# PM25/Information-Retrieval-with-Contrastive-Learning

Hardware: AMD Instinct MI355X
Metric: query-doc pairs/sec (train) + queries/sec @ top-k over N docs, 1/2/4/8 GPU (higher is better)
Workload: dtype bf16

## Files before the change

### information-retrieval-with-contrastive-learning_amd/csrc/gemm.hip

```cpp
#include "gemm_epi.h"
#include "gemm_pp.h"

#include <algorithm>
#include <atomic>
#include <type_traits>

#ifndef IRC_GEMM_GROUP_M
#define IRC_GEMM_GROUP_M 0
#endif

namespace irc {
namespace gemm {

enum Layout { ROW = 0, COL = 1 };

constexpr int BM = 128, BN = 128, NT = 256;

template <typename T>
struct TT;
template <>
struct TT<unsigned short> {
  static constexpr int BK = 32;
  static constexpr int VEC = 8;
  static constexpr int PITCH = BK * 2 + 16;
// ... 1090 lines not shown
        if (EPI == EPI_BIAS_GELU_SAVE) {
          TO* pre = const_cast<TO*>(R) + (int64_t)row * g.ldr + col;
          if constexpr (sizeof(TO) == 2)
            *reinterpret_cast<unsigned short*>(pre) = f32_to_bf16(v);
          else
            *reinterpret_cast<float*>(pre) = v;
          v = gelu_fast(v);
        }
        if (EPI == EPI_BIAS_RESID || EPI == EPI_RESID || EPI == EPI_DGELU) {
          float r;
          if constexpr (sizeof(TO) == 2)
            r = bf16_to_f32(reinterpret_cast<const unsigned short*>(R)[(int64_t)row * g.ldr + col]);
          else
            r = reinterpret_cast<const float*>(R)[(int64_t)row * g.ldr + col];
          v = EPI == EPI_DGELU ? v * gelu_grad_fast(r) : v + r;
        }
        TO* dst = C + (int64_t)row * g.ldc + col;
        if constexpr (sizeof(TO) == 2) {
          *reinterpret_cast<unsigned short*>(dst) = f32_to_bf16(v);
        } else {
          if (g.accumulate)
            *reinterpret_cast<float*>(dst) += v;
          else
            *reinterpret_cast<float*>(dst) = v;
        }
      }
    }
  }
}

typedef __bf16 bf16x2_v __attribute__((ext_vector_type(2)));
struct QaArgs {
  const unsigned short* x;
  const unsigned short* w;
  const float* bias;
  const int64_t* mask;
  unsigned short* ctx;
  int M, K, H;
  int64_t ldx, ldc;
  float scale;
  int L;
  int group_m;
  int big_dma;
  int l2_touch;
};

template <int SL>
__global__ __launch_bounds__(big::NT, 1) void qkv_attn_kernel(QaArgs g) {
  constexpr bool PACK = SL == 0;
  constexpr int WNB = 3, BM = big::BM, BN = 128 * WNB, TP = BN + 8;
  constexpr int SLX = PACK ? 128 : SL;
  constexpr int SH = SLX == 64 ? 6 : 7;
  constexpr int NJM = SLX / 32;
  __shared__ __attribute__((aligned(1024))) char lds[2 * (BM + BN) * big::ROW_BYTES];
  static_assert(128 * TP * 2 + 8 * SLX * 4 <= 2 * (BM + BN) * big::ROW_BYTES,
                "staged half and mask biases fit the LDS");
  const int nseq = g.M / g.L;
  const int spt = PACK ? BM / g.L : BM / SLX;
  const int ls = PACK || g.L == SL ? 0 : g.L;
  const int tiles_m = (nseq + spt - 1) / spt;
  const int tiles_n = 3 * g.H / BN;
  const int ntiles = tiles_m * tiles_n;
  int bid = blockIdx.x;
  {
    const int q = ntiles / 8, r = ntiles % 8, x = bid % 8;
    bid = (x < r ? x * (q + 1) : r * (q + 1) + (x - r) * q) + bid / 8;
  }
  int tm, tn;
  grouped_tile(bid, tiles_m, tiles_n, g.group_m, tm, tn);
  const int m0 = PACK ? tm * spt * g.L : tm * BM, n0 = tn * BN;
  const int lane = threadIdx.x & 63;
  const int wave = __builtin_amdgcn_readfirstlane(threadIdx.x >> 6);
  const int wm = wave >> 2, wn = wave & 3;
  f32x4 acc4[8][2 * WNB];
#pragma unroll
  for (int i = 0; i < 8; ++i)
#pragma unroll
    for (int j = 0; j < 2 * WNB; ++j) acc4[i][j] = (f32x4)0.0f;
  big::mainloop_mf16<WNB>(g.x, g.ldx, g.w, g.K, m0, n0, g.M, 3 * g.H, g.K, lds, wave, lane, acc4,
                          g.big_dma != 0,
                          big::touch_lines(g.l2_touch, tiles_m, tiles_n, tm, tn, BM, BN), ls, SH);

  unsigned short* T = reinterpret_cast<unsigned short*>(lds);
  float* mbw = reinterpret_cast<float*>(lds + 128 * TP * 2) + SL * wave;
  uint32_t pk[8][2 * WNB][2];
#pragma unroll
  for (int j = 0; j < 2 * WNB; ++j) {
    const int col = n0 + wn * 32 * WNB + 16 * j + (lane & 15);
    const float bvj = g.bias[col];
#pragma unroll
    for (int i = 0; i < 8; ++i)
#pragma unroll
      for (int e2 = 0; e2 < 2; ++e2) {
        f32x2_t v;
#pragma unroll
        for (int u = 0; u < 2; ++u) v[u] = acc4[i][j][2 * e2 + u] * 1.0f + bvj;
        uint32_t w = __builtin_bit_cast(uint32_t, __builtin_convertvector(v, bf16x2_v));
        asm volatile("" : "+v"(w));
        pk[i][j][e2] = w;
      }
  }
  const int h = lane >> 5, r32 = lane & 31;
  const int nj = (g.L + 31) / 32;
  if constexpr (PACK) {
    constexpr int TQ = 264;
    static_assert(BM * TQ * 2 + 8 * 128 * 4 <= 2 * (BM + BN) * big::ROW_BYTES,
                  "staged head and mask biases fit the LDS");
    unsigned short* Tq = reinterpret_cast<unsigned short*>(lds);
    float* mb = reinterpret_cast<float*>(lds + BM * TQ * 2) + 128 * wave;
    const int odd = lane & 1;
    const uint32_t psel = odd ? 0x03020706u : 0x05040100u;
    const int nsq = min(spt, nseq - tm * spt);
    const int nit = nsq * nj;
#pragma unroll
    for (int hd = 0; hd < 2; ++hd) {
#pragma unroll
      for (int j = 0; j < 2 * WNB; ++j) {
        const int b = wn * 32 * WNB + 16 * j;
        if (((b >> 6) & 1) != hd) continue;
        const int tc = 64 * (b >> 7) + (b & 63) + (lane & 14);
#pragma unroll
        for (int i = 0; i < 8; ++i)
#pragma unroll
          for (int e2 = 0; e2 < 2; ++e2) {
            const uint32_t w = pk[i][j][e2];
            const uint32_t x = (uint32_t)__builtin_amdgcn_mov_dpp((int)w, 0xB1, 0xF, 0xF, false);
            const uint32_t v = __builtin_amdgcn_perm(x, w, psel);
            const int rl = 128 * wm + 16 * i + 4 * (lane >> 4) + 2 * e2 + odd;
            *reinterpret_cast<uint32_t*>(&Tq[rl * TQ + tc]) = v;
          }
      }
      __syncthreads();
      for (int it = wave; it < nit; it += 8) {
        const int s = it / nj, ib = it - s * nj;
        const int t0 = s * g.L;
        const int r0 = (tm * spt + s) * g.L;
#pragma unroll
        for (int j = lane; j < 128; j += 64)
          mb[j] = j >= g.L ? -3e30f
                           : ((g.mask == nullptr || g.mask[r0 + j] != 0) ? 0.f : -1e30f);
        const int nkb = visible_key_blocks(g.mask ? g.mask + r0 : nullptr, g.L, nj, lane);
        __builtin_amdgcn_wave_barrier();
        asm volatile("s_waitcnt lgkmcnt(0)" ::: "memory");
        const unsigned short* Q = Tq;
        const unsigned short* Kp = Tq + 64;
        const unsigned short* V = Tq + 128;
        unsigned short* out = g.ctx + (int64_t)r0 * g.ldc + (2 * tn + hd) * 64;
        bf16x8 qf[4];
        const int qr = min(t0 + 32 * ib + r32, BM - 1);
#pragma unroll
        for (int kk = 0; kk < 4; ++kk)
          qf[kk] = *reinterpret_cast<const bf16x8*>(Q + qr * TQ + 16 * kk + 8 * h);
        f32x16 sc[NJM];
#pragma unroll
        for (int jb = 0; jb < NJM; ++jb) {
          sc[jb] = (f32x16)0.f;
          if (jb < nkb) {
            const int kr = min(t0 + 32 * jb + r32, BM - 1);
#pragma unroll
            for (int kk = 0; kk < 4; ++kk) {
              const bf16x8 kf = *reinterpret_cast<const bf16x8*>(Kp + kr * TQ + 16 * kk + 8 * h);
              sc[jb] = __builtin_amdgcn_mfma_f32_32x32x16_bf16(kf, qf[kk], sc[jb], 0, 0, 0);
            }
          }
        }
        float mx = -INFINITY;
#pragma unroll
        for (int jb = 0; jb < NJM; ++jb) {
          if (jb >= nkb) break;
#pragma unroll
          for (int q = 0; q < 4; ++q) {
            const f32x4 bias = *reinterpret_cast<const f32x4*>(&mb[32 * jb + 8 * q + 4 * h]);
#pragma unroll
            for (int r = 0; r < 4; ++r) {
              const float v = sc[jb][4 * q + r] * g.scale + bias[r];
              sc[jb][4 * q + r] = v;
              mx = fmaxf(mx, v);
            }
          }
        }
        mx = fmaxf(mx, __shfl_xor(mx, 32, 64));
        float sum = 0.f;
#pragma unroll
        for (int jb = 0; jb < NJM; ++jb) {
          if (jb >= nkb) break;
#pragma unroll
          for (int e = 0; e < 16; ++e) {
            const float p = __expf(sc[jb][e] - mx);
            sc[jb][e] = p;
            sum += p;
          }
        }
        sum += __shfl_xor(sum, 32, 64);
        const float inv = 1.f / sum;
        f32x16 o[2] = {(f32x16)0.f, (f32x16)0.f};
#pragma unroll
        for (int jb = 0; jb < NJM; ++jb) {
          if (jb >= nkb) break;
#pragma unroll
          for (int k2 = 0; k2 < 2; ++k2) {
            bf16x8 pa;
#pragma unroll
            for (int t = 0; t < 8; ++t) pa[t] = (__bf16)(sc[jb][8 * k2 + t] * inv);
            const int j0 = 32 * jb + 16 * k2 + 4 * h;
            const int i16 = lane & 15;
            const int vr = t0 + j0 + (i16 >> 2);
#pragma unroll
            for (int db = 0; db < 2; ++db) {
              const int vc = 32 * db + 16 * ((lane >> 4) & 1) + 4 * (i16 & 3);
              const v4s lo = ds_tr16(reinterpret_cast<const char*>(V + min(vr, BM - 1) * TQ + vc));
              const v4s hi =
                  ds_tr16(reinterpret_cast<const char*>(V + min(vr + 8, BM - 1) * TQ + vc));
              const v4s both[2] = {lo, hi};
              o[db] = __builtin_amdgcn_mfma_f32_32x32x16_bf16(pa, __builtin_bit_cast(bf16x8, both),
                                                              o[db], 0, 0, 0);
            }
          }
        }
#pragma unroll
        for (int db = 0; db < 2; ++db)
#pragma unroll
          for (int e = 0; e < 16; ++e) {
            const int i = 32 * ib + (e & 3) + 8 * (e >> 2) + 4 * h;
            if (i < g.L) out[(int64_t)i * g.ldc + 32 * db + r32] = f32_to_bf16(o[db][e]);
          }
      }
      if (hd == 0) __syncthreads();
    }
    return;
  }
#pragma unroll
  for (int hf = 0; hf < 2; ++hf) {
    if (wm == hf) {
      const int odd = lane & 1;
      const uint32_t psel = odd ? 0x03020706u : 0x05040100u;
#pragma unroll
      for (int i = 0; i < 8; ++i)
#pragma unroll
        for (int j = 0; j < 2 * WNB; ++j)
#pragma unroll
          for (int e2 = 0; e2 < 2; ++e2) {
            const uint32_t w = pk[i][j][e2];
            const uint32_t x = (uint32_t)__builtin_amdgcn_mov_dpp((int)w, 0xB1, 0xF, 0xF, false);
            const uint32_t v = __builtin_amdgcn_perm(x, w, psel);
            const int rl = 16 * i + 4 * (lane >> 4) + 2 * e2 + odd;
            *reinterpret_cast<uint32_t*>(&T[rl * TP + wn * 32 * WNB + 16 * j + (lane & 14)]) = v;
          }
    }
    __syncthreads();
    const int sl = SL == 64 ? wn >> 1 : 0, hh = SL == 64 ? wn & 1 : wave & 1;
    const int ib = SL == 64 ? wm : wave >> 1;
    const int seq = spt * tm + (SL == 64 ? 2 * hf + sl : hf);
    const int r0 = seq * g.L;
    if (seq < nseq && ib < nj) {
#pragma unroll
      for (int j = lane; j < SL; j += 64)
        mbw[j] = j >= g.L ? -3e30f
                          : ((g.mask == nullptr || g.mask[r0 + j] != 0) ? 0.f : -1e30f);
      const int nkb = visible_key_blocks(g.mask ? g.mask + r0 : nullptr, g.L, nj, lane);
      __builtin_amdgcn_wave_barrier();
      asm volatile("s_waitcnt lgkmcnt(0)" ::: "memory");
      const unsigned short* Ts = T + 64 * sl * TP;
      const unsigned short* Q = Ts + hh * 64;
      const unsigned short* Kp = Ts + 128 + hh * 64;
      const unsigned short* V = Ts + 256 + hh * 64;
      unsigned short* out = g.ctx + (int64_t)r0 * g.ldc + (2 * tn + hh) * 64;
      {
        bf16x8 qf[4];
#pragma unroll
        for (int kk = 0; kk < 4; ++kk)
          qf[kk] = *reinterpret_cast<const bf16x8*>(Q + (32 * ib + r32) * TP + 16 * kk + 8 * h);
        f32x16 sc[NJM];
#pragma unroll
        for (int jb = 0; jb < NJM; ++jb) {
          sc[jb] = (f32x16)0.f;
          if (jb < nkb) {
#pragma unroll
            for (int kk = 0; kk < 4; ++kk) {
              const bf16x8 kf =
                  *reinterpret_cast<const bf16x8*>(Kp + (32 * jb + r32) * TP + 16 * kk + 8 * h);
              sc[jb] = __builtin_amdgcn_mfma_f32_32x32x16_bf16(kf, qf[kk], sc[jb], 0, 0, 0);
            }
          }
        }
        float mx = -INFINITY;
#pragma unroll
        for (int jb = 0; jb < NJM; ++jb) {
          if (jb >= nkb) break;
#pragma unroll
          for (int q = 0; q < 4; ++q) {
            const f32x4 bias = *reinterpret_cast<const f32x4*>(&mbw[32 * jb + 8 * q + 4 * h]);
#pragma unroll
            for (int r = 0; r < 4; ++r) {
              const float v = sc[jb][4 * q + r] * g.scale + bias[r];
              sc[jb][4 * q + r] = v;
              mx = fmaxf(mx, v);
            }
          }
        }
        mx = fmaxf(mx, __shfl_xor(mx, 32, 64));
        float sum = 0.f;
#pragma unroll
        for (int jb = 0; jb < NJM; ++jb) {
          if (jb >= nkb) break;
#pragma unroll
          for (int e = 0; e < 16; ++e) {
            const float p = __expf(sc[jb][e] - mx);
            sc[jb][e] = p;
            sum += p;
          }
        }
        sum += __shfl_xor(sum, 32, 64);
        const float inv = 1.f / sum;
        f32x16 o[2] = {(f32x16)0.f, (f32x16)0.f};
#pragma unroll
        for (int jb = 0; jb < NJM; ++jb) {
          if (jb >= nkb) break;
#pragma unroll
          for (int k2 = 0; k2 < 2; ++k2) {
            bf16x8 pa;
#pragma unroll
            for (int t = 0; t < 8; ++t) pa[t] = (__bf16)(sc[jb][8 * k2 + t] * inv);
            const int j0 = 32 * jb + 16 * k2 + 4 * h;
#pragma unroll
            for (int db = 0; db < 2; ++db) {
              const int i16 = lane & 15;
              const unsigned short* vp =
                  V + (j0 + (i16 >> 2)) * TP + 32 * db + 16 * ((lane >> 4) & 1) + 4 * (i16 & 3);
              const v4s lo = ds_tr16(reinterpret_cast<const char*>(vp));
              const v4s hi = ds_tr16(reinterpret_cast<const char*>(vp + 8 * TP));
              const v4s both[2] = {lo, hi};
              o[db] = __builtin_amdgcn_mfma_f32_32x32x16_bf16(pa, __builtin_bit_cast(bf16x8, both),
                                                              o[db], 0, 0, 0);
            }
          }
        }
#pragma unroll
        for (int db = 0; db < 2; ++db)
#pragma unroll
          for (int e = 0; e < 16; ++e) {
            const int i = 32 * ib + (e & 3) + 8 * (e >> 2) + 4 * h;
            if (i < g.L) out[(int64_t)i * g.ldc + 32 * db + r32] = f32_to_bf16(o[db][e]);
          }
      }
    }
    if (hf == 0) __syncthreads();
  }
}

inline int big_wnb(const Args& g, int batch, int la, int lb) {
  if (la != ROW || lb != ROW || !g.vec_a || !g.vec_b) return 0;
  if (g.K % big::BK != 0 || g.K == 0) return 0;
  const int wnb = g.N % 384 == 0 ? 3 : 2;
  const int64_t tiles = (int64_t)((g.M + 255) / 256) * ((g.N + 128 * wnb - 1) / (128 * wnb)) * batch;
  return tiles >= 128 ? wnb : 0;
}

template <typename TO, int EPI, bool LN = false>
static int launch_big(const Args& g0, int batch, int wnb, hipStream_t st) {
  Args g = g0;
  g.big_dma = big_dma_flag(g.M, g.N, g.K, g.lda, g.ldb);
  const int bn = 128 * wnb;
  g.l2_touch = l2_touch_flag(g.big_dma, g.group_m, (g.N + bn - 1) / bn);
  const int tiles = ((g.M + big::BM - 1) / big::BM) * ((g.N + bn - 1) / bn);
  prof_begin(st);
  const bool ring = big_ring() && g.K % big::BK4 == 0;
  if constexpr (LN) {
    if (wnb == 3)
      hipLaunchKernelGGL((gemm_big_kernel<TO, EPI, 3, false, true, true>), dim3(tiles, batch), dim3(big::NT), 0, st, g);
    else
      hipLaunchKernelGGL((gemm_big_kernel<TO, EPI, 2, false, true, true>), dim3(tiles, batch), dim3(big::NT), 0, st, g);
  } else if (big_mf16() && !ring) {
    if (wnb == 3)
      hipLaunchKernelGGL((gemm_big_kernel<TO, EPI, 3, false, true>), dim3(tiles, batch), dim3(big::NT), 0, st, g);
    else
      hipLaunchKernelGGL((gemm_big_kernel<TO, EPI, 2, false, true>), dim3(tiles, batch), dim3(big::NT), 0, st, g);
  } else if (wnb == 3 && ring)
    hipLaunchKernelGGL((gemm_big_kernel<TO, EPI, 3, true>), dim3(tiles, batch), dim3(big::NT), 0, st, g);
  else if (wnb == 3)
    hipLaunchKernelGGL((gemm_big_kernel<TO, EPI, 3>), dim3(tiles, batch), dim3(big::NT), 0, st, g);
  else if (ring)
    hipLaunchKernelGGL((gemm_big_kernel<TO, EPI, 2, true>), dim3(tiles, batch), dim3(big::NT), 0, st, g);
  else
    hipLaunchKernelGGL((gemm_big_kernel<TO, EPI, 2>), dim3(tiles, batch), dim3(big::NT), 0, st, g);
  prof_end("gemm_bf16", st, 2.0 * g.M * g.N * g.K * batch);
  prof_work("gemm_bf16_bytes", gemm_alg_bytes(sizeof(TO) == 4, EPI, g.accumulate, g.M, g.N, g.K,
                                               batch));
  return check_launch("gemm_big_kernel");
}

template <typename TI, typename TO, int LA, int LB, int EPI>
static int launch(const Args& g0, int batch, int splits, hipStream_t st) {
  if constexpr (sizeof(TI) == 2) {
    if (splits == 1) {
      const int wnb = big_wnb(g0, batch, LA, LB);
      if (wnb) return launch_big<TO, EPI>(g0, batch, wnb, st);
    }
  }
  Args g = g0;
  const int tiles = ((g.M + BM - 1) / BM) * ((g.N + BN - 1) / BN);
  constexpr int bk = TT<TI>::BK;
  g.kchunk = splits > 1 ? ((g.K + splits - 1) / splits + bk - 1) / bk * bk : (g.K > 0 ? g.K : 1);
  prof_begin(st);
  hipLaunchKernelGGL((gemm_kernel<TI, TO, LA, LB, EPI>), dim3(tiles, batch, splits), dim3(NT), 0,
                     st, g);
  if (splits > 1) {
    const int64_t n = (int64_t)g.M * g.N * batch;
    hipLaunchKernelGGL(splitk_reduce_kernel, dim3((unsigned)((n + 255) / 256)), dim3(256), 0, st,
                       g.P, reinterpret_cast<float*>(g.C), g.M, g.N, splits, g.ldc, g.sC, batch,
                       g.alpha, g.accumulate, EPI == EPI_BIAS ? g.bias : nullptr, g.sBias);
  }
  prof_end(sizeof(TI) == 2 ? "gemm_bf16" : "gemm_f32", st, 2.0 * g.M * g.N * g.K * batch);
  if (sizeof(TI) == 2)
    prof_work("gemm_bf16_bytes", gemm_alg_bytes(sizeof(TO) == 4, EPI, g.accumulate, g.M, g.N, g.K,
                                                 batch));
  return check_launch("gemm_kernel");
}

template <typename TI, typename TO, int LA, int LB>
static int by_epi(int epi, const Args& g, int batch, int splits, hipStream_t st) {
  switch (epi) {
    case EPI_NONE: return launch<TI, TO, LA, LB, EPI_NONE>(g, batch, splits, st);
    case EPI_BIAS:
      return launch<TI, TO, LA, LB, EPI_BIAS>(g, batch, sizeof(TI) == 4 ? splits : 1, st);
    case EPI_BIAS_GELU: return launch<TI, TO, LA, LB, EPI_BIAS_GELU>(g, batch, 1, st);
    case EPI_BIAS_RESID: return launch<TI, TO, LA, LB, EPI_BIAS_RESID>(g, batch, 1, st);
// ... 306 lines not shown
```

### information-retrieval-with-contrastive-learning_amd/csrc/gemm_pp.hip

```cpp
#include "gemm_epi.h"
#include "gemm_pp.h"
#include "mx.h"

#include <atomic>
#include <cstdlib>
#include <mutex>

namespace irc {
namespace gpp {
using namespace irc::gemm;

#ifdef IRC_SCAN_STAMPS
__device__ uint64_t pp_stamps[16];
#define PSTAMP(i)                                                              \
  do {                                                                         \
    if (blockIdx.x == 0 && threadIdx.x == 0)                                   \
      *(volatile uint64_t*)&pp_stamps[(i) + (int)(threadIdx.x & 0)] =          \
          __builtin_amdgcn_s_memrealtime();                                    \
  } while (0)
#else
#define PSTAMP(i) \
  do {            \
  } while (0)
#endif

constexpr int BM = 256, BN = 256, BK = 64, NT = 512;
constexpr int BPITCH = 1024 + 64;
constexpr int slot_bytes(bool kmajor) { return kmajor ? 16384 : 16 * BPITCH; }
constexpr int buf_bytes(bool ak, bool bk) { return 2 * slot_bytes(ak) + 2 * slot_bytes(bk); }
constexpr int LDS_BYTES = 2 * buf_bytes(false, false);
constexpr int EP_PITCH = 68;

template <bool KMAJOR>
__device__ __forceinline__ void stage_half(const unsigned short* __restrict__ X, int64_t ld,
                                           int r0, int nrows, int k0, char* img, int wq,
                                           int lane) {
#pragma unroll
  for (int i = 0; i < 4; ++i) {
    const int p = (i * 4 + wq) * 64 + lane;
    if constexpr (KMAJOR) {
      const int row = p >> 3;
      const int c = (p & 7) ^ (row & 7);
      int gr = r0 + row;
      gr = gr < nrows ? gr : nrows - 1;
      glds16(X + (int64_t)gr * ld + k0 + c * 8, img + (i * 4 + wq) * 1024);
    } else {
      const int blk = i * 4 + wq;
      const int a = lane >> 4;
      int gc = r0 + ((lane & 15) ^ (2 * a)) * 8;
      gc = gc + 8 <= nrows ? gc : nrows - 8;
      glds16(X + (int64_t)(k0 + 4 * blk + a) * ld + gc, img + blk * BPITCH);
    }
  }
}

template <bool KMAJOR>
__device__ __forceinline__ bf16x8 frag(const char* img, int row0, int s, int lane) {
  if constexpr (KMAJOR) {
    const int row = row0 + (lane & 15);
    const int c = 4 * s + (lane >> 4);
    return *reinterpret_cast<const bf16x8*>(img + row * 128 + 16 * (c ^ (row & 7)));
  } else {
    const int q = lane >> 4, a = (lane >> 2) & 3, b = lane & 3;
    const int col = row0 + 4 * b;
    const char* p =
        img + (8 * s + 2 * q) * BPITCH + a * 256 + (((col >> 3) ^ (2 * a)) * 16) + (col & 7) * 2;
    const v4s lo = ds_tr16(p);
    const v4s hi = ds_tr16(p + BPITCH);
    const v4s both[2] = {lo, hi};
    return __builtin_bit_cast(bf16x8, both);
  }
}

typedef int v8i32 __attribute__((ext_vector_type(8)));

template <int OA, int OB>
__device__ __forceinline__ f32x4 mfma_mx(v8i32 a, v8i32 b, f32x4 c, int sa, int sb) {
  return __builtin_amdgcn_mfma_scale_f32_16x16x128_f8f6f4(a, b, c, 0, 0, OA, sa, OB, sb);
}
__device__ __forceinline__ f32x4 mfma_mx_sel(int oa, int ob, v8i32 a, v8i32 b, f32x4 c, int sa,
                                             int sb) {
  switch (oa * 4 + ob) {
#define IRC_MXS(OA, OB) \
  case OA * 4 + OB:     \
    return mfma_mx<OA, OB>(a, b, c, sa, sb);
    IRC_MXS(0, 0) IRC_MXS(0, 1) IRC_MXS(0, 2) IRC_MXS(0, 3)
    IRC_MXS(1, 0) IRC_MXS(1, 1) IRC_MXS(1, 2) IRC_MXS(1, 3)
    IRC_MXS(2, 0) IRC_MXS(2, 1) IRC_MXS(2, 2) IRC_MXS(2, 3)
    IRC_MXS(3, 0) IRC_MXS(3, 1) IRC_MXS(3, 2)
// ... 307 lines not shown
#pragma unroll
              for (int t = 0; t < 8; ++t) v[t] += bf16_to_f32(rr[t]);
            }
          }
          if (EPI == EPI_BIAS_GELU_SAVE) {
            u16x8 pre;
#pragma unroll
            for (int t = 0; t < 8; t += 2) {
              pre[t] = f32_to_bf16(v[t]);
              pre[t + 1] = f32_to_bf16(v[t + 1]);
              const f32x2_t g2 = gelu_f2(f32x2_t{v[t], v[t + 1]});
              v[t] = g2.x;
              v[t + 1] = g2.y;
            }
            *reinterpret_cast<u16x8*>(const_cast<unsigned short*>(R) + (int64_t)row * g.ldr + col) =
                pre;
          }
          if (F8 == 2 && g.cx != nullptr) {
            uint2 q8;
#pragma unroll
            for (int t = 0; t < 8; ++t) v[t] = bf16_to_f32(f32_to_bf16(v[t]));
            const unsigned e8 = mx_quant8(v, q8);
            unsigned char* C8 = reinterpret_cast<unsigned char*>(g.C);
            *reinterpret_cast<uint2*>(C8 + (int64_t)row * g.ldc + col) = q8;
            if ((lane & 3) == 0) g.cx[mx_scale_index(row, col, g.mpad)] = (unsigned char)e8;
            continue;
          }
          u16x8 o;
#pragma unroll
          for (int t = 0; t < 8; ++t) o[t] = f32_to_bf16(v[t]);
          if (lnout) {
            float s1 = 0.f, s2 = 0.f;
#pragma unroll
            for (int t = 0; t < 8; ++t) {
              const float x = bf16_to_f32(o[t]);
              s1 += x;
              s2 = __builtin_fmaf(x, x, s2);
            }
            const int lr = row - m0;
            atomicAdd(&lst[2 * lr], s1);
            atomicAdd(&lst[2 * lr + 1], s2);
          }
#ifdef IRC_PP_DIAG_NOSTORE
          if (o[0] == 0x7fc1 && o[7] == 0x7fc3)
#endif
          *reinterpret_cast<u16x8*>(C + (int64_t)row * g.ldc + col) = o;
        }
      } else {
        const float* R = reinterpret_cast<const float*>(g.R) + batch * g.sR;
        float* C = reinterpret_cast<float*>(g.C) + batch * g.sC;
#pragma unroll
        for (int it = 0; it < 8; ++it) {
          const int c = it * 64 + lane;
          const int rl = c >> 4, c4 = (c & 15) * 4;
          const int row = rbase + rl, col = cbase + c4;
          if (row >= g.M || col >= g.N) continue;
          f32x4 v = *reinterpret_cast<const f32x4*>(&st[rl * EP_PITCH + c4]);
          if (EPI == EPI_BIAS_RESID || EPI == EPI_RESID || EPI == EPI_DGELU) {
            const f32x4 r = *reinterpret_cast<const f32x4*>(R + (int64_t)row * g.ldr + col);
#pragma unroll
            for (int t = 0; t < 4; ++t) v[t] = EPI == EPI_DGELU ? v[t] * gelu_grad_fast(r[t]) : v[t] + r[t];
          }
          if (EPI == EPI_BIAS_GELU_SAVE) {
            *reinterpret_cast<f32x4*>(const_cast<float*>(R) + (int64_t)row * g.ldr + col) = v;
#pragma unroll
            for (int t = 0; t < 4; ++t) v[t] = gelu_fast(v[t]);
          }
          float* dst = C + (int64_t)row * g.ldc + col;
          if (g.accumulate) v += *reinterpret_cast<const f32x4*>(dst);
          *reinterpret_cast<f32x4*>(dst) = v;
        }
      }
      __builtin_amdgcn_wave_barrier();
      asm volatile("s_waitcnt lgkmcnt(0)" ::: "memory");
    }
    if (lnout) {
      lds_barrier();
      const int lr = threadIdx.x >> 1, row = m0 + lr;
      if (row < g.M)
        g.ln.st_out[((int64_t)row * g.ln.nt_out + n0 / BN) * 2 + (threadIdx.x & 1)] = lst[threadIdx.x];
    }
    return;
  }
}

template <typename Fn>
__device__ __forceinline__ void epilogue_scan(const PArgs& g, const f32x4 (&acc)[8][4], char* lds,
                                              int m0, int n0, int tn, int grp, int wn, int lane,
                                              Fn after_init) {
  const int cbase = n0 + 64 * wn;
  PSTAMP(1);
  uint32_t* cnt = reinterpret_cast<uint32_t*>(lds);
  uint64_t* thk = reinterpret_cast<uint64_t*>(lds + 1024);
  float* thf = reinterpret_cast<float*>(lds + 3072);
  if (threadIdx.x < 256) {
    const int q = m0 + threadIdx.x;
    const uint64_t t = (g.thr != nullptr && q < g.M) ? g.thr[q] : 0ull;
    cnt[threadIdx.x] = 0;
    thk[threadIdx.x] = t;
    const uint32_t hi = (uint32_t)(t >> 32);
    thf[threadIdx.x] = q >= g.M ? __builtin_huge_valf()
                                : (hi == 0 ? -__builtin_huge_valf() : unorderable_f32(hi));
  }
  lds_barrier();
  after_init();
#ifdef IRC_PP_SCAN_NOEPI
  if (threadIdx.x < 256 && m0 + (int)threadIdx.x < g.qpad)
    g.counts[(int64_t)tn * g.qpad + m0 + threadIdx.x] = acc[0][0][0] == 12345.f ? 1u : 0u;
  return;
#endif
  float* slotv = reinterpret_cast<float*>(lds + 4096) + threadIdx.x * 32;
  const int sw = (lane >> 1) & 7;
  uint64_t pm[2] = {0, 0};
  const float* thq = thf + 128 * grp + 4 * (lane >> 4);
#pragma unroll
  for (int i = 0; i < 8; ++i) {
    const f32x4 tf = *reinterpret_cast<const f32x4*>(&thq[16 * i]);
#pragma unroll
    for (int j = 0; j < 4; ++j)
#pragma unroll
      for (int e = 0; e < 4; ++e) {
        const int bit = 16 * i + 4 * j + e;
        pm[bit >> 6] |= (uint64_t)(!(acc[i][j][e] < tf[e])) << (bit & 63);
      }
  }
  PSTAMP(2);
#pragma unroll
  for (int qq = 0; qq < 4; ++qq) {
    uint32_t bits = (uint32_t)(pm[qq >> 1] >> (32 * (qq & 1)));
    if (__ballot(bits != 0) == 0) continue;
#pragma unroll
    for (int i = 0; i < 2; ++i)
#pragma unroll
      for (int j = 0; j < 4; ++j)
        *reinterpret_cast<f32x4*>(slotv + 4 * ((4 * i + j) ^ sw)) = acc[2 * qq + i][j];
    while (__ballot(bits != 0) != 0) {
      if (bits != 0) {
        const int b = __builtin_ctz(bits);
        bits &= bits - 1;
        const float v = slotv[4 * ((b >> 2) ^ sw) + (b & 3)];
        const int bit = 32 * qq + b;
        const int ql = 128 * grp + 16 * (bit >> 4) + 4 * (lane >> 4) + (bit & 3);
        const int q = m0 + ql;
        const int d = cbase + 16 * ((bit >> 2) & 3) + (lane & 15);
        if (q < g.M && d < g.N) {
          const uint64_t key = make_key(v, g.idx_base + (uint32_t)d * (uint32_t)g.stride);
          if (key >= thk[ql]) {
            const uint32_t slot = atomicAdd(&cnt[ql], 1u);
            g.keys[((int64_t)tn * g.qpad + q) * g.cap + slot] = key;
          }
        }
      }
    }
  }
  PSTAMP(3);
  lds_barrier();
  PSTAMP(4);
  if (threadIdx.x < 256 && m0 + (int)threadIdx.x < g.qpad)
    g.counts[(int64_t)tn * g.qpad + m0 + threadIdx.x] = cnt[threadIdx.x];
}

__device__ __forceinline__ bool top_better(float va, int ia, float vb, int ib) {
  return va > vb || (va == vb && ia < ib);
}
__device__ __forceinline__ void top_cswap(float& va, int& ia, float& vb, int& ib) {
  const bool sw = top_better(vb, ib, va, ia);
// ... 283 lines not shown
    }
    lds_barrier();
  }
}

template <bool AK, bool BK_, typename TO, int EPI, int F8 = 0, bool LN = false>
__global__ __launch_bounds__(NT, 1) void gemm_pp_kernel(PArgs g) {
  __shared__ __attribute__((aligned(1024))) char lds[LDS_BYTES];
  const int tiles_m = (g.M + BM - 1) / BM;
  const int tiles_n = (g.N + BN - 1) / BN;
  const int ntiles = tiles_m * tiles_n;
  int bid, batch, split;
  {
    const int nz = gridDim.y * gridDim.z;
    const int total = ntiles * nz;
    const int lin = blockIdx.x + gridDim.x * (blockIdx.y + gridDim.y * blockIdx.z);
    const int q = total / 8, r = total % 8, x = lin % 8;
    const int w = (x < r ? x * (q + 1) : r * (q + 1) + (x - r) * q) + lin / 8;
    bid = w % ntiles;
    const int rest = w / ntiles;
    split = rest % gridDim.z;
    batch = rest / gridDim.z;
  }
  int tm, tn;
  if (EPI == EPI_SCAN || EPI == EPI_PICK || EPI == EPI_GROUP) {
    tm = bid % tiles_m;
    tn = bid / tiles_m;
  } else {
    grouped_tile(bid, tiles_m, tiles_n, g.group_m, tm, tn);
  }
  const int kbeg = split * g.kchunk;
  const int kend = min(g.K, kbeg + g.kchunk);
  const int nk = (kend - kbeg) / BK;
  const unsigned short* A = g.A + batch * g.sA;
  const unsigned short* B = g.B + batch * g.sB;
  const int m0 = tm * BM, n0 = tn * BN;
  const int lane = threadIdx.x & 63;
  const int wave = __builtin_amdgcn_readfirstlane(threadIdx.x >> 6);
  const int grp = wave >> 2, wq = wave & 3;
  const int wn = wq;

  if (EPI == EPI_SCAN) PSTAMP(0);
  if constexpr (EPI == EPI_PICK) {
    static_assert(AK && BK_ && F8 != 2, "the pick ranges live past two K-major buffers");
    if (!pick_ranges(g, lds, m0, n0)) return;
  }
  if constexpr (EPI == EPI_GROUP) {
    static_assert(AK && BK_ && F8 != 2, "the group map lives past two K-major buffers");
    if (!group_map(g, lds, n0)) return;
  }
  f32x4 acc[8][4];
  mainloop<AK, BK_, F8>(g, A, B, m0, n0, kbeg, nk, lds, buf_bytes(AK, BK_), 0, false, acc, grp,
                        wq, lane, nullptr, 0);

  const int rbase0 = m0 + 128 * grp;
  const int cbase = n0 + 64 * wn;
  if constexpr (EPI == EPI_SCAN) {
    if (g.lists != nullptr)
      epilogue_scan_lists(g, acc, lds, m0, n0, tn, grp, wn, lane, [] {});
    else
      epilogue_scan(g, acc, lds, m0, n0, tn, grp, wn, lane, [] {});
    return;
  }
  if constexpr (EPI == EPI_PICK) {
    epilogue_pick<F8>(g, acc, lds, m0, n0, grp, wn, lane);
    return;
  }
  if constexpr (EPI == EPI_GROUP) {
    epilogue_group<F8>(g, acc, lds, m0, n0, grp, wn, lane);
    return;
  }
#ifdef IRC_PP_DIAG_NOEPI
  {
    float t = 0.f;
#pragma unroll
    for (int i = 0; i < 8; ++i)
#pragma unroll
      for (int j = 0; j < 4; ++j) t += acc[i][j][0] + acc[i][j][1] + acc[i][j][2] + acc[i][j][3];
    if (t == 1234.5f) reinterpret_cast<float*>(g.C)[threadIdx.x] = t;
    return;
  }
#endif
  if (g.P != nullptr || g.vec_c) {
    epilogue_vec<TO, EPI, F8, LN>(g, acc, lds, m0, n0, batch, grp, wn, wave, lane, split);
    return;
  }
  const float* bias = g.bias ? g.bias + batch * g.sBias : nullptr;
  const TO* R = reinterpret_cast<const TO*>(g.R) + (g.R ? batch * g.sR : 0);
  TO* C = reinterpret_cast<TO*>(g.C) + batch * g.sC;
#pragma unroll
  for (int j = 0; j < 4; ++j) {
    const int col = cbase + 16 * j + (lane & 15);
    if (col >= g.N) continue;
    const float bvv = epi_has_bias(EPI) ? bias[col] : 0.f;
#pragma unroll
    for (int i = 0; i < 8; ++i)
#pragma unroll
      for (int e = 0; e < 4; ++e) {
        const int row = rbase0 + 16 * i + 4 * (lane >> 4) + e;
        if (row >= g.M) continue;
        float v = acc[i][j][e] * g.alpha + bvv;
        if (EPI == EPI_BIAS_GELU) v = sizeof(TO) == 2 ? gelu_lite(v) : gelu_fast(v);
        if (EPI == EPI_BIAS_GELU_SAVE) {
          TO* pre = const_cast<TO*>(R) + (int64_t)row * g.ldr + col;
          if constexpr (sizeof(TO) == 2)
            *reinterpret_cast<unsigned short*>(pre) = f32_to_bf16(v);
          else
            *reinterpret_cast<float*>(pre) = v;
          v = gelu_fast(v);
        }
        if (EPI == EPI_BIAS_RESID || EPI == EPI_RESID || EPI == EPI_DGELU) {
          float r;
          if constexpr (sizeof(TO) == 2)
            r = bf16_to_f32(reinterpret_cast<const unsigned short*>(R)[(int64_t)row * g.ldr + col]);
          else
            r = reinterpret_cast<const float*>(R)[(int64_t)row * g.ldr + col];
          v = EPI == EPI_DGELU ? v * gelu_grad_fast(r) : v + r;
        }
        TO* dst = C + (int64_t)row * g.ldc + col;
        if constexpr (sizeof(TO) == 2) {
          *reinterpret_cast<unsigned short*>(dst) = f32_to_bf16(v);
        } else {
          if (g.accumulate)
            *reinterpret_cast<float*>(dst) += v;
          else
            *reinterpret_cast<float*>(dst) = v;
        }
      }
  }
}

constexpr int PBUF = 8 * 32 * EP_PITCH * 4;
static_assert(PBUF >= buf_bytes(false, false) && 2 * PBUF <= LDS_BYTES, "persistent LDS plan");

template <bool AK, bool BK_, typename TO, int EPI, int F8 = 0>
__global__ __launch_bounds__(NT, 1) void gemm_pp_pers_kernel(PArgs g, uint32_t* ctr, int mode) {
  __shared__ __attribute__((aligned(1024))) char lds[LDS_BYTES];
  __shared__ int s_next;
  const int tiles_m = (g.M + BM - 1) / BM, tiles_n = (g.N + BN - 1) / BN;
  const int ntiles = tiles_m * tiles_n;
  auto tile_m = [&](int t) {
    int tm, tn;
    grouped_tile(t, tiles_m, tiles_n, g.group_m, tm, tn);
    return EPI == EPI_SCAN ? t % tiles_m : tm;
  };
  auto tile_n = [&](int t) {
    int tm, tn;
    grouped_tile(t, tiles_m, tiles_n, g.group_m, tm, tn);
    return EPI == EPI_SCAN ? t / tiles_m : tn;
  };
  const int G = gridDim.x;
  int slot;
  {
    const int q = G / 8, r = G % 8, x = blockIdx.x % 8;
    slot = (x < r ? x * (q + 1) : r * (q + 1) + (x - r) * q) + blockIdx.x / 8;
  }
  int tile = slot;
  const bool dyn = mode == 1, pre = mode != 3;
  const int lane = threadIdx.x & 63;
  const int wave = __builtin_amdgcn_readfirstlane(threadIdx.x >> 6);
  const int grp = wave >> 2, wq = wave & 3;
  const int nk = g.K / BK;
  int pending = G + slot;
  if (dyn && threadIdx.x == 0) pending = G + (int)atomicAdd(ctr, 1u);
  if (pre)
    stage_tile<AK, BK_>(g, g.A, g.B, tile_m(tile) * BM, tile_n(tile) * BN, 0, lds + PBUF, grp, wq,
                        lane);
  f32x4 acc[8][4];
  while (true) {
    int ln = lane;
    asm volatile("" : "+v"(ln));
    const int tn = tile_n(tile);
    const int m0 = tile_m(tile) * BM, n0 = tn * BN;
    mainloop<AK, BK_, F8>(g, g.A, g.B, m0, n0, 0, nk, lds, PBUF, 1, pre, acc, grp, wq, ln,
                          dyn ? &s_next : nullptr, pending);
    int next;
    if (dyn) {
      next = __builtin_amdgcn_readfirstlane(s_next);
      if (next < ntiles && threadIdx.x == 0) pending = G + (int)atomicAdd(ctr, 1u);
    } else {
      next = tile + G;
    }
    auto prestage = [&] {
      if (pre && next < ntiles)
        stage_tile<AK, BK_>(g, g.A, g.B, tile_m(next) * BM, tile_n(next) * BN, 0, lds + PBUF, grp,
                            wq, ln);
    };
    if constexpr (EPI == EPI_SCAN) {
      if (g.lists != nullptr)
        epilogue_scan_lists(g, acc, lds, m0, n0, tn, grp, wq, ln, prestage);
      else
        epilogue_scan(g, acc, lds, m0, n0, tn, grp, wq, ln, prestage);
    } else {
      prestage();
      epilogue_vec<TO, EPI, F8>(g, acc, lds, m0, n0, 0, grp, wq, wave, ln);
    }
    if (next >= ntiles) break;
    tile = next;
    if (!pre) wg_barrier();
  }
  if (dyn && threadIdx.x == 0 && atomicAdd(ctr + 1, 1u) == (uint32_t)G - 1) {
    atomicExch(ctr, 0u);
    atomicExch(ctr + 1, 0u);
  }
}

}

namespace gpp {

template <bool AK, bool BKM, typename TO>
static void launch_epi(int epi, const PArgs& a, dim3 grid, hipStream_t st) {
  switch (epi) {
#define IRC_PP(E)                                                                           \
  case E:                                                                                   \
    hipLaunchKernelGGL((gemm_pp_kernel<AK, BKM, TO, E>), grid, dim3(NT), 0, st, a); \
    break;
    IRC_PP(0) IRC_PP(1) IRC_PP(2) IRC_PP(3) IRC_PP(4) IRC_PP(5) IRC_PP(6)
#undef IRC_PP
  }
}

template <typename TO>
static void launch_layout(int la, int lb, int epi, const PArgs& a, dim3 grid, hipStream_t st);

extern "C" int irc_pp_dbg_stamps(uint64_t* out ) {
#ifdef IRC_SCAN_STAMPS
  if (hipDeviceSynchronize() != hipSuccess) return -1;
  return hipMemcpyFromSymbol(out, HIP_SYMBOL(pp_stamps), sizeof(pp_stamps)) == hipSuccess ? 0 : -1;
#else
  (void)out;
  return -1;
#endif
}

static std::atomic<int>& pers_mode() {
  static std::atomic<int> on{0};
  return on;
}
static bool pers_enabled() { return pers_mode().load(std::memory_order_relaxed) != 0; }

int cu_count() {
  static int cus[64] = {};
  int dev = 0;
  if (hipGetDevice(&dev) != hipSuccess || dev < 0 || dev >= 64) return 0;
  if (cus[dev] == 0) {
    int n = 0;
    if (hipDeviceGetAttribute(&n, hipDeviceAttributeMultiprocessorCount, dev) != hipSuccess) n = -1;
    cus[dev] = n;
  }
  return cus[dev];
}

constexpr int PERS_SLOTS = 1024;
static uint32_t* pers_counter(hipStream_t st) {
  hipStreamCaptureStatus cap = hipStreamCaptureStatusNone;
  if (hipStreamIsCapturing(st, &cap) != hipSuccess || cap != hipStreamCaptureStatusNone)
    return nullptr;
  static std::mutex mu;
  static uint32_t* base[64] = {};
  static std::atomic<uint32_t> next{0};
  int dev = 0;
  if (hipGetDevice(&dev) != hipSuccess || dev < 0 || dev >= 64) return nullptr;
  {
    std::lock_guard<std::mutex> lk(mu);
    if (base[dev] == nullptr) {
      void* p = nullptr;
      if (hipMalloc(&p, PERS_SLOTS * 64) != hipSuccess) return nullptr;
      if (hipMemset(p, 0, PERS_SLOTS * 64) != hipSuccess || hipDeviceSynchronize() != hipSuccess) {
        (void)hipFree(p);
        return nullptr;
      }
      base[dev] = static_cast<uint32_t*>(p);
    }
  }
  return base[dev] + (next.fetch_add(1) % PERS_SLOTS) * 16;
}

// ... 194 lines not shown
```

Before: 34810.

## Hoist attention mask preprocessing, pack context stores, add specialized fp32 GEMM epilogue

In the fused QKV+attention kernel, the key-padding mask is now loaded once per sequence before the head loop. It is converted to additive biases and visible-key-block counts in shared LDS, so each wave no longer re-reads the mask and recomputes block counts. Context outputs are written as packed bf16 pairs, using DPP swaps between neighbouring lanes, whenever the pointer and stride are aligned. Separately, a new fp32-output epilogue for the persistent GEMM stages tiles through LDS, prefetches residual and accumulate operands ahead, and writes f32x4 vectors. This adds code complexity and LDS layout assumptions.

```diff
diff --git a/information-retrieval-with-contrastive-learning_amd/csrc/gemm.hip b/information-retrieval-with-contrastive-learning_amd/csrc/gemm.hip
--- a/information-retrieval-with-contrastive-learning_amd/csrc/gemm.hip
+++ b/information-retrieval-with-contrastive-learning_amd/csrc/gemm.hip
@@ -1196,7 +1196,6 @@
                           big::touch_lines(g.l2_touch, tiles_m, tiles_n, tm, tn, BM, BN), ls, SH);
 
   unsigned short* T = reinterpret_cast<unsigned short*>(lds);
-  float* mbw = reinterpret_cast<float*>(lds + 128 * TP * 2) + SL * wave;
   uint32_t pk[8][2 * WNB][2];
 #pragma unroll
   for (int j = 0; j < 2 * WNB; ++j) {
@@ -1206,9 +1205,7 @@
     for (int i = 0; i < 8; ++i)
 #pragma unroll
       for (int e2 = 0; e2 < 2; ++e2) {
-        f32x2_t v;
-#pragma unroll
-        for (int u = 0; u < 2; ++u) v[u] = acc4[i][j][2 * e2 + u] * 1.0f + bvj;
+        const f32x2_t v = f32x2_t{acc4[i][j][2 * e2], acc4[i][j][2 * e2 + 1]} + f32x2_t{bvj, bvj};
         uint32_t w = __builtin_bit_cast(uint32_t, __builtin_convertvector(v, bf16x2_v));
         asm volatile("" : "+v"(w));
         pk[i][j][e2] = w;
@@ -1343,6 +1340,18 @@
     }
     return;
   }
+  constexpr int SPT = PACK ? 1 : BM / SLX, MW = PACK ? 1 : SL / 64;
+  float* mbs = reinterpret_cast<float*>(lds + 128 * TP * 2);
+  int* nkbs = reinterpret_cast<int*>(mbs + SPT * SL);
+  static_assert(PACK || SPT * SL + SPT <= 8 * SL, "bias rows and counts fit the mask area");
+  const bool mrow = wave < SPT && spt * tm + wave < nseq;
+  int64_t mraw[MW];
+#pragma unroll
+  for (int c = 0; c < MW; ++c) {
+    const int j = lane + 64 * c;
+    mraw[c] = (mrow && g.mask != nullptr && j < g.L) ? g.mask[(spt * tm + wave) * g.L + j] : 1;
+  }
+  const bool ctx2 = (((uintptr_t)g.ctx & 3) | (g.ldc & 1)) == 0;
 #pragma unroll
   for (int hf = 0; hf < 2; ++hf) {
     if (wm == hf) {
@@ -1361,19 +1370,29 @@
             *reinterpret_cast<uint32_t*>(&T[rl * TP + wn * 32 * WNB + 16 * j + (lane & 14)]) = v;
           }
     }
+    if (hf == 0 && mrow) {
+      int last = -1;
+#pragma unroll
+      for (int c = 0; c < MW; ++c) {
+        const int j = lane + 64 * c;
+        const bool vis = j < g.L && mraw[c] != 0;
+        mbs[wave * SL + j] = j >= g.L ? -3e30f : (vis ? 0.f : -1e30f);
+        const uint64_t b = __ballot(vis);
+        if (b != 0) last = 64 * c + 63 - __builtin_clzll(b);
+      }
+#ifdef IRC_ATTN_NO_SKIP
+      last = -1;
+#endif
+      if (lane == 0) nkbs[wave] = last < 0 ? nj : last / 32 + 1;
+    }
     __syncthreads();
     const int sl = SL == 64 ? wn >> 1 : 0, hh = SL == 64 ? wn & 1 : wave & 1;
     const int ib = SL == 64 ? wm : wave >> 1;
     const int seq = spt * tm + (SL == 64 ? 2 * hf + sl : hf);
     const int r0 = seq * g.L;
     if (seq < nseq && ib < nj) {
-#pragma unroll
-      for (int j = lane; j < SL; j += 64)
-        mbw[j] = j >= g.L ? -3e30f
-                          : ((g.mask == nullptr || g.mask[r0 + j] != 0) ? 0.f : -1e30f);
-      const int nkb = visible_key_blocks(g.mask ? g.mask + r0 : nullptr, g.L, nj, lane);
-      __builtin_amdgcn_wave_barrier();
-      asm volatile("s_waitcnt lgkmcnt(0)" ::: "memory");
+      const float* mbw = mbs + (seq - spt * tm) * SL;
+      const int nkb = __builtin_amdgcn_readfirstlane(nkbs[seq - spt * tm]);
       const unsigned short* Ts = T + 64 * sl * TP;
       const unsigned short* Q = Ts + hh * 64;
       const unsigned short* Kp = Ts + 128 + hh * 64;
@@ -1449,13 +1468,31 @@
             }
           }
         }
-#pragma unroll
-        for (int db = 0; db < 2; ++db)
-#pragma unroll
-          for (int e = 0; e < 16; ++e) {
-            const int i = 32 * ib + (e & 3) + 8 * (e >> 2) + 4 * h;
-            if (i < g.L) out[(int64_t)i * g.ldc + 32 * db + r32] = f32_to_bf16(o[db][e]);
-          }
+        if (ctx2) {
+          const int odd = lane & 1;
+          const uint32_t psel = odd ? 0x03020706u : 0x05040100u;
+          unsigned short* op = out + 32 * ib * g.ldc + (4 * h + odd) * g.ldc + (r32 & 30);
+#pragma unroll
+          for (int db = 0; db < 2; ++db)
+#pragma unroll
+            for (int e = 0; e < 16; e += 2) {
+              const uint32_t w = __builtin_bit_cast(
+                  uint32_t, __builtin_convertvector(f32x2_t{o[db][e], o[db][e + 1]}, bf16x2_v));
+              const uint32_t x = (uint32_t)__builtin_amdgcn_mov_dpp((int)w, 0xB1, 0xF, 0xF, false);
+              const uint32_t v = __builtin_amdgcn_perm(x, w, psel);
+              const int i = 32 * ib + (e & 3) + 8 * (e >> 2) + 4 * h + odd;
+              if (i < g.L)
+                *reinterpret_cast<uint32_t*>(op + ((e & 3) + 8 * (e >> 2)) * g.ldc + 32 * db) = v;
+            }
+        } else {
+#pragma unroll
+          for (int db = 0; db < 2; ++db)
+#pragma unroll
+            for (int e = 0; e < 16; ++e) {
+              const int i = 32 * ib + (e & 3) + 8 * (e >> 2) + 4 * h;
+              if (i < g.L) out[(int64_t)i * g.ldc + 32 * db + r32] = f32_to_bf16(o[db][e]);
+            }
+        }
       }
     }
     if (hf == 0) __syncthreads();
diff --git a/information-retrieval-with-contrastive-learning_amd/csrc/gemm_pp.hip b/information-retrieval-with-contrastive-learning_amd/csrc/gemm_pp.hip
--- a/information-retrieval-with-contrastive-learning_amd/csrc/gemm_pp.hip
+++ b/information-retrieval-with-contrastive-learning_amd/csrc/gemm_pp.hip
@@ -5,6 +5,7 @@
 #include <atomic>
 #include <cstdlib>
 #include <mutex>
+#include <type_traits>
 
 namespace irc {
 namespace gpp {
@@ -478,6 +479,18 @@
     }
     return;
   }
+}
+
+#include "gemm_pp_epi_f32.h"
+
+template <typename TO, int EPI, int F8, bool LN>
+__device__ __forceinline__ void epilogue_tile(const PArgs& g, const f32x4 (&acc)[8][4], char* lds,
+                                              int m0, int n0, int batch, int grp, int wn, int wave,
+                                              int lane, int split) {
+  if constexpr (sizeof(TO) == 4 && F8 == 0 && !LN)
+    epilogue_f32<EPI>(g, acc, lds, m0, n0, batch, grp, wn, wave, lane, split);
+  else
+    epilogue_vec<TO, EPI, F8, LN>(g, acc, lds, m0, n0, batch, grp, wn, wave, lane, split);
 }
 
 template <typename Fn>
@@ -927,7 +940,7 @@
   }
 #endif
   if (g.P != nullptr || g.vec_c) {
-    epilogue_vec<TO, EPI, F8, LN>(g, acc, lds, m0, n0, batch, grp, wn, wave, lane, split);
+    epilogue_tile<TO, EPI, F8, LN>(g, acc, lds, m0, n0, batch, grp, wn, wave, lane, split);
     return;
   }
   const float* bias = g.bias ? g.bias + batch * g.sBias : nullptr;
@@ -1038,7 +1051,7 @@
         epilogue_scan(g, acc, lds, m0, n0, tn, grp, wq, ln, prestage);
     } else {
       prestage();
-      epilogue_vec<TO, EPI, F8>(g, acc, lds, m0, n0, 0, grp, wq, wave, ln);
+      epilogue_tile<TO, EPI, F8, false>(g, acc, lds, m0, n0, 0, grp, wq, wave, ln, 0);
     }
     if (next >= ntiles) break;
     tile = next;
diff --git a/information-retrieval-with-contrastive-learning_amd/csrc/gemm_pp_epi_f32.h b/information-retrieval-with-contrastive-learning_amd/csrc/gemm_pp_epi_f32.h
--- /dev/null
+++ b/information-retrieval-with-contrastive-learning_amd/csrc/gemm_pp_epi_f32.h
@@ -0,0 +1,156 @@
+#pragma once
+
+template <int EPI>
+__device__ __forceinline__ void epilogue_f32(const PArgs& g, const f32x4 (&acc)[8][4], char* lds,
+                                             int m0, int n0, int batch, int grp, int wn, int wave,
+                                             int lane, int split) {
+  constexpr bool READS_R = EPI == EPI_BIAS_RESID || EPI == EPI_RESID || EPI == EPI_DGELU;
+  constexpr bool USES_R = READS_R || EPI == EPI_BIAS_GELU_SAVE;
+  const int rbase0 = m0 + 128 * grp;
+  const int cbase = n0 + 64 * wn;
+  float* st = reinterpret_cast<float*>(lds) + wave * (32 * EP_PITCH);
+  const bool slab = EPI == EPI_NONE && g.P != nullptr;
+  float* C = slab ? g.P + ((int64_t)batch * gridDim.z + split) * g.M * g.N
+                  : reinterpret_cast<float*>(g.C) + batch * g.sC;
+  const float* R = reinterpret_cast<const float*>(g.R) + batch * g.sR;
+  const int64_t ldc = slab ? (int64_t)g.N : g.ldc;
+  const int64_t ldr = g.ldr;
+  const bool accum = !slab && g.accumulate != 0;
+  const bool cvec = !slab || (g.N & 3) == 0;
+  const bool fast = m0 + BM <= g.M && n0 + BN <= g.N && cvec && ldc < (1 << 24) &&
+                    (!USES_R || ldr < (1 << 24));
+  const float* bias = g.bias ? g.bias + batch * g.sBias : nullptr;
+  float bv[4];
+#pragma unroll
+  for (int j = 0; j < 4; ++j) {
+    const int col = cbase + 16 * j + (lane & 15);
+    bv[j] = (!slab && epi_has_bias(EPI) && col < g.N) ? bias[col] : 0.f;
+  }
+  const float alpha1 = slab ? 1.f : g.alpha;
+  const f32x2_t alpha = {alpha1, alpha1};
+  float* sw = st + 4 * (lane >> 4) * EP_PITCH + (lane & 15);
+
+  auto finish = [&](f32x4 v, const f32x4& r, const float* rp) -> f32x4 {
+    if constexpr (READS_R) {
+#pragma unroll
+      for (int t = 0; t < 4; ++t) v[t] = EPI == EPI_DGELU ? v[t] * gelu_grad_fast(r[t]) : v[t] + r[t];
+    }
+    if constexpr (EPI == EPI_BIAS_GELU_SAVE) {
+      *reinterpret_cast<f32x4*>(const_cast<float*>(rp)) = v;
+#pragma unroll
+      for (int t = 0; t < 4; ++t) v[t] = gelu_fast(v[t]);
+    }
+    return v;
+  };
+  auto stage = [&](int p) {
+#pragma unroll
+    for (int ii = 0; ii < 2; ++ii)
+#pragma unroll
+      for (int j = 0; j < 4; ++j) {
+        const f32x4& a = acc[2 * p + ii][j];
+        f32x2_t v0 = __builtin_elementwise_fma(f32x2_t{a[0], a[1]}, alpha, f32x2_t{bv[j], bv[j]});
+        f32x2_t v1 = __builtin_elementwise_fma(f32x2_t{a[2], a[3]}, alpha, f32x2_t{bv[j], bv[j]});
+        if constexpr (EPI == EPI_BIAS_GELU) {
+          v0 = gelu_f2(v0);
+          v1 = gelu_f2(v1);
+        }
+        float* d = sw + 16 * ii * EP_PITCH + 16 * j;
+        d[0] = v0.x;
+        d[EP_PITCH] = v0.y;
+        d[2 * EP_PITCH] = v1.x;
+        d[3 * EP_PITCH] = v1.y;
+      }
+    __builtin_amdgcn_wave_barrier();
+    asm volatile("s_waitcnt lgkmcnt(0)" ::: "memory");
+  };
+  auto staged = [&]() {
+    __builtin_amdgcn_wave_barrier();
+    asm volatile("s_waitcnt lgkmcnt(0)" ::: "memory");
+  };
+
+  if (fast) {
+    uint32_t soff = 0, coff = 0, roff = 0;
+    auto set_offsets = [&]() {
+      int ln = lane;
+      asm volatile("" : "+v"(ln));
+      const int rl0 = ln >> 4, c4 = (ln & 15) * 4;
+      soff = rl0 * EP_PITCH + c4;
+      coff = 4u * (uint32_t)(rl0 * (int)ldc + c4);
+      roff = USES_R ? 4u * (uint32_t)(rl0 * (int)ldr + c4) : 0u;
+    };
+    auto passes = [&](auto acc_c) {
+      constexpr bool ACC = decltype(acc_c)::value;
+      f32x4 rq[8], cq[8];
+      auto load_ahead = [&](int p, int it) {
+        const int64_t row = rbase0 + 32 * p + 4 * it;
+        if constexpr (READS_R)
+          rq[it] = *reinterpret_cast<const f32x4*>(
+              reinterpret_cast<const char*>(R + row * ldr + cbase) + roff);
+        if constexpr (ACC)
+          cq[it] = *reinterpret_cast<const f32x4*>(
+              reinterpret_cast<const char*>(C + row * ldc + cbase) + coff);
+      };
+#pragma unroll
+      for (int p = 0; p < 4; ++p) {
+        stage(p);
+        if (p == 0) {
+          set_offsets();
+          if constexpr (READS_R || ACC) {
+#pragma unroll
+            for (int it = 0; it < 8; ++it) load_ahead(0, it);
+          }
+        }
+        char* cu = reinterpret_cast<char*>(C + (int64_t)(rbase0 + 32 * p) * ldc + cbase);
+        const char* ru = reinterpret_cast<const char*>(R + (int64_t)(rbase0 + 32 * p) * ldr + cbase);
+#pragma unroll
+        for (int it = 0; it < 8; ++it) {
+          f32x4 v = *reinterpret_cast<const f32x4*>(st + soff + 4 * it * EP_PITCH);
+          f32x4 r = {};
+          if constexpr (READS_R) r = rq[it];
+          v = finish(v, r, reinterpret_cast<const float*>(ru + 16 * it * ldr + roff));
+          if constexpr (ACC) v += cq[it];
+#ifdef IRC_PP_DIAG_NOSTORE
+          if (v[0] == 1234.5f && v[3] == 5432.1f)
+#endif
+          *reinterpret_cast<f32x4*>(cu + 16 * it * ldc + coff) = v;
+          if constexpr (READS_R || ACC) {
+            if (p < 3) load_ahead(p + 1, it);
+          }
+        }
+        staged();
+      }
+    };
+    if (accum) passes(std::true_type{});
+    else passes(std::false_type{});
+    return;
+  }
+
+#pragma unroll
+  for (int p = 0; p < 4; ++p) {
+    stage(p);
+    const int rbase = rbase0 + 32 * p;
+#pragma unroll
+    for (int it = 0; it < 8; ++it) {
+      const int c = it * 64 + lane;
+      const int rl = c >> 4, c4 = (c & 15) * 4;
+      const int row = rbase + rl, col = cbase + c4;
+      if (row >= g.M || col >= g.N) continue;
+      f32x4 v = *reinterpret_cast<const f32x4*>(&st[rl * EP_PITCH + c4]);
+      float* dst = C + (int64_t)row * ldc + col;
+      if (!cvec) {
+        for (int t = 0; t < 4 && col + t < g.N; ++t) dst[t] = v[t];
+        continue;
+      }
+      const float* rp = R + (int64_t)row * ldr + col;
+      f32x4 r = {};
+      if constexpr (READS_R) r = *reinterpret_cast<const f32x4*>(rp);
+      v = finish(v, r, rp);
+      if (accum) v += *reinterpret_cast<const f32x4*>(dst);
+#ifdef IRC_PP_DIAG_NOSTORE
+      if (v[0] == 1234.5f && v[3] == 5432.1f)
+#endif
+      *reinterpret_cast<f32x4*>(dst) = v;
+    }
+    staged();
+  }
+}
```

Result: no change. 35070 (median of 6 runs) (+0.7%).
